# bharatlytics/faceRecognition_InfrenceEngine

Hardware: AMD Instinct MI355X
Metric: faces/sec end-to-end @1080p (higher is better)
Workload: dtype f16

## Files before the change

facerecognition_infrenceengine_amd/_lib.py:

```python
import ctypes as C
import struct
import os
import threading

_HERE = os.path.dirname(os.path.abspath(__file__))
LIB_PATH = os.path.join(_HERE, "csrc", "libfrhip.so")

_lock = threading.Lock()
_lib = None
ABI_VERSION = 106


class FrError(RuntimeError):
    pass


class ConvArgs(C.Structure):
    _fields_ = [("x", C.c_void_p), ("w", C.c_void_p), ("y", C.c_void_p),
                ("bias", C.c_void_p), ("slope", C.c_void_p), ("residual", C.c_void_p),
                ("out_f32_partial", C.c_void_p),
                ("B", C.c_int), ("H", C.c_int), ("W", C.c_int), ("Cin", C.c_int), ("Cout", C.c_int),
                ("KH", C.c_int), ("KW", C.c_int), ("stride", C.c_int), ("pad", C.c_int),
                ("Ho", C.c_int), ("Wo", C.c_int), ("bias_mode", C.c_int), ("splitk", C.c_int),
                ("x2", C.c_void_p), ("C2", C.c_int)]
# ... 63 lines not shown
    "fr_gallery_match_grouped_workspace": (_Z, [_I, _L]),
    "fr_gallery_match_grouped_f32": (_I, [_P, _P, _P, _P, _P, _I, _I, _L, _L, _I, _P, _P, _P, _Z, _P, _I, _P]),
    "fr_gallery_topk_grouped_workspace": (_Z, [_I, _L, _I]),
    "fr_gallery_topk_grouped_f32": (_I, [_P, _P, _P, _P, _P, _I, _I, _L, _L, _I, _I, _P, _P, _P, _Z, _P, _I, _P]),
    "fr_gallery_gmax_update": (_I, [_P, _P, _L, _I, _P, _P]),
    "fr_f32_to_f8": (_I, [_P, _P, _L, _P]),
    "fr_f32_to_f16": (_I, [_P, _P, _L, _P]),
    "fr_match_decide": (_I, [_P, _P, _I, _F, _F, _P, _P]),
    "fr_match_pack_candidates": (_I, [_P, _P, _I, _P, _P]),
    "fr_match_reduce_shards": (_I, [_P, _I, _I, _I, _I, _P, _P, _P]),
    "fr_match_reduce_shards_topk": (_I, [_P, _I, _I, _I, _I, _I, _P, _P, _P]),
    "fr_exchange_pack_queries": (_I, [_P, _I, _I, _I, _P, _P]),
    "fr_exchange_counts": (_I, [_P, _I, _I, _I, _P, _P]),
    "fr_gallery_first_above_f32": (_I, [_P, _P, _I, _L, _I, _F, _I, _L, _P, _P, _P, _Z, _P]),
    "fr_cosine_matrix_f32": (_I, [_P, _P, _I, _I, _I, _P, _P]),
    "fr_mean_rows_f32": (_I, [_P, _I, _I, _P, _P]),
    "fr_unknown_assign_batch_f32": (_I, [_P, _P, _I, _I, _F, _P, _P, _P, _I, _I, _P, _P, _P, _P]),
    "fr_gallery_first_above_blocked_f32": (_I, [_P, _P, _P, _P, _I, _L, _I, _F, _I, _L, _P, _P, _P, _Z, _P]),
    "fr_enrol_batch_workspace": (_Z, [_I, _L]),
    "fr_enrol_batch_f32": (_I, [_P, _P, _I, _P, _P, _I, _P, _I, _I, _I, _P, _P, _L, _F, _F, _P, _P, _P, _P, _P, _P, _P, _P,
                                _Z, _P]),
    "fr_gallery_pairs_workspace": (_Z, [_L, _L]),
    "fr_gallery_pairs_above_f16": (_I, [_P, _P, _L, _I, _F, _I, _L, _I, _P, _P, _P, _P, _Z, _P]),
    "fr_conv_nhwc_f16": (_I, [C.POINTER(ConvArgs), _P]),
    "fr_conv_sequence": (_I, [C.POINTER(ConvStep), _I, _P]),
    "fr_conv_inblock_f16": (_I, [C.POINTER(ConvArgs), _P]),
    "fr_conv_nhwc_f8": (_I, [C.POINTER(ConvF8Args), _P]),
    "fr_quantize_f16_f8": (_I, [_P, _P, _L, _F, _P]),
    "fr_quantize_f16_f8_centred": (_I, [_P, _P, _L, _I, _P, _F, _P]),
    "fr_gptq_round_e4m3": (_I, [_P, _P, _P, _P, _I, _I, _P]),
    "fr_conv_stage14_weight_bytes": (_Z, [_I]),
    "fr_conv_stage14_pack": (_I, [_P, _P, _P]),
    "fr_conv_stage14_f16": (_I, [_P, _P, _P, _P, _I, _I, _P]),
    "fr_conv_walk64_weight_bytes": (_Z, [_I]),
    "fr_conv_walk64_pack": (_I, [_P, _P, _I, _P]),
    "fr_conv_walk64_f16": (_I, [_P, _P, _P, _P, _I, _P, _P, _I, _I, _I, _P]),
    "fr_conv_stage28_weight_bytes": (_Z, [_I]),
    "fr_conv_stage28_pack": (_I, [_P, _P, _P]),
    "fr_conv_stage28_f16": (_I, [_P, _P, _P, _P, _I, _I, _P]),
    "fr_conv_stage14_f8_weight_bytes": (_Z, [_I]),
    "fr_conv_stage14_f8_param_floats": (_Z, []),
    "fr_conv_stage14_f8_pack": (_I, [_P, _P, _P]),
    "fr_conv_stage14_f8": (_I, [_P, _P, _P, _P, _P, _I, _I, _P]),
    "fr_conv_splitk_epilogue": (_I, [_P, _I, _I, _I, _I, _I, _P, _I, _P, _P, _P, _P]),
    "fr_fc_reduce_l2norm": (_I, [_P, _I, _I, _I, _P, _P, _P, _P]),
    "fr_warp_affine_5pt": (_I, [_P, _I, _I, _I, _P, _P, _P, _I, _I, _P, _P, _P, _P]),
    "fr_warp_affine_5pt_slots": (_I, [_P, _I, _I, _I, _P, _P, _I, _I, _P, _P]),
    "fr_warp_affine_5pt_refs": (_I, [_P, _I, _P, _P, _P, _I, _I, _P, _P, _P, _P]),
    "fr_warp_affine_5pt_slots_refs": (_I, [_P, _I, _P, _P, _I, _I, _P, _P]),
    "fr_letterbox_u8": (_I, [_P, _I, _P, _I, _I, _P]),
    "fr_detections_unscale": (_I, [_P, _P, _P, _P, _I, _I, _P]),
    "fr_yuv420_to_bgr_u8": (_I, [_P, _P, _I, _I, _I, _I, _I, _I, _I, _I, _I, _I, _P]),
    "fr_yuv420_to_bgr_refs_u8": (_I, [_P, _P, _I, _I, _I, _I, _I, _I, _I, _I, _P]),
    "fr_frame_activity_u8": (_I, [_P, _I, _I, _I, _P, _I, _P, _P, _P, _I, _P, _P, _P, _I, _I, _I, _P]),
    "fr_frame_activity_refs_u8": (_I, [_P, _I, _P, _I, _P, _P, _P, _I, _P, _P, _P, _I, _I, _I, _P]),
    "fr_track_associate_f32": (_I, [_P, _P, _P, _I, _I, _I, _I, _P, _P, _P, _F, _I, _I, _P, _P, _P, _P]),
    "fr_track_commit_f32": (_I, [_P, _P, _P, _P, _I, _I, _I, _I, _P, _P, _P, _P]),
    "fr_track_resolve_quality_i32": (_I, [_P, _P, _P, _P, _P, _P, _I, _I, _I, _I, _P, _P, _I, _P, _P, _P, _P]),
    "fr_track_fuse_f32": (_I, [_P, _P, _P, _P, _P, _P, _I, _I, _I, _I, _I, _F, _P, _P, _P, _P, _P, _P, _P]),
    "fr_face_quality_f16": (_I, [_P, _P, _P, _I, _I, _P, _P, _P, _F, _I, _I, _I, _I, _I, _F, _F, _F, _P]),
    "fr_pyramid_resize_norm":(_I, [_P, _I, _I, _I, _I, _I, _P, _P]),
    "fr_dconv_f32": (_I, [_P, _P, _P, _P, _P, _I, _I, _I, _I, _I, _I, _I, _I, _I, _P, _P, _I, _P]),
    "fr_dconv_mfma_f32": (_I, [_I, _P, _P, _P, _P, _P, _I, _I, _I, _P, _P, _P, _I, _I, _P, _I, _P, _P]),
    "fr_crop_conv1_f32": (_I, [_I, _P, _I, _I, _I, _P, _P, _I, _P, _P, _P, _P, _P]),
    "fr_crop_conv1_split": (_I, [_I, _P, _I, _I, _I, _P, _P, _I, _P, _P, _P, _P, _I, _P]),
    "fr_crop_conv1_list_f32": (_I, [_I, _P, _I, _I, _I, _P, _I, _P, _P, _I, _P, _P, _P, _P, _P]),
# ... 148 lines not shown
```

facerecognition_infrenceengine_amd/csrc/conv_stage14.hip:

```cpp
#include "common.h"
#include <type_traits>

namespace {

constexpr int S14_PX = 196, S14_C = 256, S14_ROWS = 200;
constexpr int S14_PLANE = S14_ROWS * 128;
constexpr int S14_IMG = 4 * S14_PLANE;
constexpr int S14_SLOT = 256 * 64;
constexpr int S14_PRM = 10 * 256 * 4;
constexpr int S14_LDS = S14_IMG + 3 * S14_SLOT + S14_PRM;
constexpr int S14_STEPS = 72;

struct StageP {
    const half_t* x;
    half_t* y;
    const half_t* w;
    const float* prm;
    int B, nconv;
    unsigned xbytes, wbytes;
};

}

__global__ __launch_bounds__(512, 2) void conv_stage14_kernel(StageP p) {
#if defined(__HIP_DEVICE_COMPILE__)
    extern __shared__ __attribute__((aligned(16))) char lds[];
    char* img = lds;
    char* ring = lds + S14_IMG;
    const float* lprm = reinterpret_cast<const float*>(lds + S14_IMG + 3 * S14_SLOT);
    const int tid = threadIdx.x, lane = tid & 63;
    const int wave = __builtin_amdgcn_readfirstlane(tid >> 6);
    const int wn = wave & 3, wp = wave >> 2;
    const int fr = lane & 15, fq = lane >> 4;
    const int n = blockIdx.x;
    const size_t img_elems = (size_t)S14_PX * S14_C;

    __amdgpu_buffer_rsrc_t wrs = buffer_rsrc(p.w, p.wbytes);
    __amdgpu_buffer_rsrc_t xrs = buffer_rsrc(p.x, p.xbytes);

    const unsigned wlane = (unsigned)(wave * 2048 + lane * 16);
    unsigned wsrc = 0;
    auto issue_w = [&](int slot) {
        char* dst = ring + slot * S14_SLOT + wave * 2048;
        __builtin_amdgcn_raw_ptr_buffer_load_lds(wrs, (lds_ptr_t)dst, 16, wlane, wsrc, 0, 0);
        __builtin_amdgcn_raw_ptr_buffer_load_lds(wrs, (lds_ptr_t)(dst + 1024), 16, wlane + 1024, wsrc, 0, 0);
        wsrc += S14_SLOT;
    };
    issue_w(0);
    issue_w(1);
    issue_w(2);
    __amdgpu_buffer_rsrc_t prs = buffer_rsrc(p.prm, (unsigned)p.nconv * S14_PRM);
    auto issue_prm = [&](int conv, int ln) {
        char* dst = lds + S14_IMG + 3 * S14_SLOT;
        __builtin_amdgcn_raw_ptr_buffer_load_lds(prs, (lds_ptr_t)(dst + wave * 1024), 16, (unsigned)(wave * 1024 + ln * 16), conv * S14_PRM, 0, 0);
        if (wave < 2)
            __builtin_amdgcn_raw_ptr_buffer_load_lds(prs, (lds_ptr_t)(dst + (8 + wave) * 1024), 16, (unsigned)((8 + wave) * 1024 + ln * 16), conv * S14_PRM, 0, 0);
    };

    {
        const int lrow = lane >> 3, ch = lane & 7;
        for (int pc = wave; pc < 100; pc += 8) {
            const int plane = pc / 25, row = (pc - plane * 25) * 8 + lrow;
            const unsigned off = row < S14_PX ? (unsigned)(((size_t)n * S14_PX + row) * 512 + plane * 128 + ((ch ^ (row & 7)) << 4))
                                              : 0x80000000u;
            __builtin_amdgcn_raw_ptr_buffer_load_lds(xrs, (lds_ptr_t)(img + plane * S14_PLANE + (pc - plane * 25) * 1024), 16, off, 0, 0, 0);
        }
    }

    auto run = [&](auto wp_tag) {
    constexpr int WP = decltype(wp_tag)::value;
    const int a_lane = fr * 64 + ((fq ^ (((fr >> 3) & 1) << 1)) << 4);
    const int a_own = wn * 4096 + a_lane;
    const int px0 = WP * 96 + fr;

    float4v acc[6][4], accx[2];
    int4v a0[4], a1[4], b[6], bx;
    int boff[7];

    int px0e = px0, fre = fr, fqe = fq;
    auto set_tap_one = [&](int j, int dy, int dx) {
        const int px = j < 6 ? px0e + 16 * j : 192 + fre;
        const int oy = px / 14, ox = px - oy * 14;
        const bool ok = px < S14_PX && (unsigned)(oy + dy) < 14u && (unsigned)(ox + dx) < 14u;
        const int pxn = ok ? px + dy * 14 + dx : S14_PX;
// ... 21 lines not shown
#pragma unroll
        for (int j = 0; j < 6; ++j) {
#pragma unroll
            for (int i = 0; i < 4; ++i) acc[j][i] = mfma16(ac[i], b[j], acc[j][i]);
            if (j == 0) { an[0] = rd_a(nslot, 0); an[1] = rd_a(nslot, 1); }
            if (j == 1) { an[2] = rd_a(nslot, 2); an[3] = rd_a(nslot, 3); }
            if (j == 2) {
                if (g == 7) { set_tap_one(6, dyn, dxn); set_tap_one(0, dyn, dxn); }
                bx = rd_b(ng, 6); b[0] = rd_b(ng, 0);
            }
            if (j == 3) {
                if (g == 7) { set_tap_one(1, dyn, dxn); set_tap_one(2, dyn, dxn); }
                b[1] = rd_b(ng, 1); b[2] = rd_b(ng, 2);
            }
            if (j == 4) {
                if (g == 7) { set_tap_one(3, dyn, dxn); set_tap_one(4, dyn, dxn); }
                b[3] = rd_b(ng, 3); b[4] = rd_b(ng, 4);
            }
            if (j == 5) {
                if (g == 7) set_tap_one(5, dyn, dxn);
                b[5] = rd_b(ng, 5);
            }
            FR_PIN();
            if constexpr (WP == 1) { if (j == 3) { issue_w(k % 3); FR_PIN(); } }
        }
    };

#pragma unroll
    for (int j = 0; j < 6; ++j)
#pragma unroll
        for (int i = 0; i < 4; ++i) acc[j][i] = float4v{0.f, 0.f, 0.f, 0.f};
    accx[0] = accx[1] = float4v{0.f, 0.f, 0.f, 0.f};
#pragma unroll 1
    for (int conv = 0; conv < p.nconv; ++conv) {
        int lane_e = lane;
        asm volatile("" : "+v"(lane_e));
        fre = lane_e & 15; fqe = lane_e >> 4; px0e = WP * 96 + fre;
        issue_prm(conv, lane_e);
        set_tap(-1, -1);
#pragma unroll
        for (int i = 0; i < 4; ++i) a0[i] = rd_a(0, i);
#pragma unroll
        for (int j = 0; j < 6; ++j) b[j] = rd_b(0, j);
        bx = rd_b(0, 6);
#pragma unroll 1
        for (int it = 0; it < 3; ++it) {
#pragma unroll
            for (int k = 0; k < 24; ++k) {
                asm volatile("s_waitcnt vmcnt(2) lgkmcnt(1)" ::: "memory");
                __builtin_amdgcn_s_barrier();
                FR_PIN();
                const int tt = k >> 3;
                const int dyn = tt < 2 ? it - 1 : it, dxn = tt < 2 ? tt : -1;
                if ((k & 1) == 0) step(a0, a1, k, dyn, dxn);
                else step(a1, a0, k, dyn, dxn);
            }
        }
        const bool second = conv & 1;
        half_t* ybase = p.y + (size_t)n * img_elems;
        asm volatile("" : "+v"(px0e), "+v"(fre), "+v"(fqe));
        asm volatile("s_waitcnt vmcnt(2)" ::: "memory");
        __builtin_amdgcn_s_barrier();
        int rowoff[7], key[7], clsoff[7];
#pragma unroll
        for (int j = 0; j < 7; ++j) {
            const int px = j < 6 ? px0e + 16 * j : 192 + fre;
            const int oy = (px * 4682) >> 16, ox = px - oy * 14;
            const int cls = (oy == 0 ? 0 : (oy >= 13 ? 2 : 1)) * 3 + (ox == 0 ? 0 : (ox == 13 ? 2 : 1));
            clsoff[j] = cls * S14_C;
            const int pxr = px < S14_PX ? px : S14_PX;
            rowoff[j] = wn * S14_PLANE + pxr * 128 + (fqe & 1) * 8;
            key[j] = pxr & 7;
        }
        const int co_own = wn * 64 + fqe * 4, co_sh = wn * 64 + WP * 32 + fqe * 4;
        const int ch_own = fqe >> 1, ch_sh = WP * 4 + (fqe >> 1);
        auto tiles = [&](auto prelu_tag) {
            constexpr bool FIRST = decltype(prelu_tag)::value;
            float4v sl[4], slx[2];
            if constexpr (FIRST) {
#pragma unroll
                for (int i = 0; i < 4; ++i) sl[i] = *reinterpret_cast<const float4v*>(lprm + 9 * S14_C + co_own + i * 16);
#pragma unroll
                for (int t = 0; t < 2; ++t) slx[t] = *reinterpret_cast<const float4v*>(lprm + 9 * S14_C + co_sh + t * 16);
            }
#pragma unroll
            for (int t = 0; t < 26; ++t) {
                float4v& a_ = t < 24 ? acc[t >> 2][t & 3] : accx[t - 24];
                const int j = t < 24 ? t >> 2 : 6, co = t < 24 ? co_own + (t & 3) * 16 : co_sh + (t - 24) * 16;
                const int ch = t < 24 ? ch_own + (t & 3) * 2 : ch_sh + (t - 24) * 2;
                half4* dst = reinterpret_cast<half4*>(img + rowoff[j] + ((ch ^ key[j]) << 4));
                float4v v = a_ + *reinterpret_cast<const float4v*>(lprm + clsoff[j] + co);
                if constexpr (FIRST) {
                    const half4 old = *dst;
                    const float4v s_ = t < 24 ? sl[t & 3] : slx[t - 24];
#pragma unroll
                    for (int e = 0; e < 4; ++e) v[e] = v[e] > 0.f ? v[e] : v[e] * s_[e];
                    a_ = float4v{(float)old[0], (float)old[1], (float)old[2], (float)old[3]};
                } else {
                    a_ = float4v{0.f, 0.f, 0.f, 0.f};
                }
                const half4 h = {(half_t)v[0], (half_t)v[1], (half_t)v[2], (half_t)v[3]};
                if (t < 24) *dst = h;
                else if (192 + fre < S14_PX) *dst = h;
                if ((t & 3) == 3) FR_PIN();
            }
        };
        if (second) tiles(std::false_type{}); else tiles(std::true_type{});
        asm volatile("s_waitcnt lgkmcnt(0)" ::: "memory");
        __builtin_amdgcn_s_barrier();
        if (conv == p.nconv - 1) {
            for (int e = tid; e < S14_PX * 32; e += 512) {
                const int px = e >> 5, c = e & 31;
                const int4v v = *reinterpret_cast<const int4v*>(img + (c >> 3) * S14_PLANE + px * 128 + (((c & 7) ^ (px & 7)) << 4));
                *reinterpret_cast<int4v*>(ybase + (size_t)px * S14_C + c * 8) = v;
            }
        }
    }
    };
    if (wp == 0) run(std::integral_constant<int, 0>{}); else run(std::integral_constant<int, 1>{});
    asm volatile("s_waitcnt vmcnt(0)" ::: "memory");
#endif
}

extern "C" size_t fr_conv_stage14_weight_bytes(int nconv) { return (size_t)(nconv > 0 ? nconv : 0) * S14_STEPS * S14_SLOT; }

__global__ void stage14_pack_weights(const half_t* __restrict__ w, half_t* __restrict__ out) {
    const int e = blockIdx.x * blockDim.x + threadIdx.x;
    if (e >= S14_STEPS * 256 * 4) return;
    const int q = e / 1024, r = e - q * 1024, row = r >> 2, cp = r & 3;
    const int chunk = cp ^ (((row >> 3) & 1) << 1);
    const int tap = q >> 3, g = q & 7;
    const int4v v = *reinterpret_cast<const int4v*>(w + (size_t)row * 2304 + tap * 256 + g * 32 + chunk * 8);
    *reinterpret_cast<int4v*>(out + (size_t)q * 8192 + row * 32 + cp * 8) = v;
}

extern "C" int fr_conv_stage14_pack(const void* w, void* out, fr_stream_t stream) {
    FR_REQUIRE(w && out, "fr_conv_stage14_pack: null pointer");
    stage14_pack_weights<<<fr_cdiv(S14_STEPS * 1024, 256), 256, 0, fr_stream(stream)>>>((const half_t*)w, (half_t*)out);
    FR_CHECK_LAUNCH("stage14_pack_weights");
    return FR_OK;
}

extern "C" int fr_conv_stage14_f16(const void* x, void* y, const void* wstream, const float* params, int B, int nblocks,
                                   fr_stream_t stream) {
    FR_REQUIRE(x && y && wstream && params && B > 0 && nblocks > 0, "fr_conv_stage14_f16: bad argument");
    FR_REQUIRE(x != y, "fr_conv_stage14_f16: x and y must be different buffers");
    FR_REQUIRE((int64_t)B * S14_PX * S14_C * 2 < (1ll << 31) && (int64_t)nblocks * 2 * S14_STEPS * S14_SLOT < (1ll << 32) - (1 << 20),
               "fr_conv_stage14_f16: tensor too large (B %d, blocks %d)", B, nblocks);
    StageP p;
    p.x = (const half_t*)x; p.y = (half_t*)y; p.w = (const half_t*)wstream; p.prm = params;
    p.B = B; p.nconv = 2 * nblocks;
    p.xbytes = (unsigned)((int64_t)B * S14_PX * S14_C * 2);
    p.wbytes = (unsigned)((int64_t)p.nconv * S14_STEPS * S14_SLOT);
    static FrDevLatch latch;
    if (!fr_raise_lds(reinterpret_cast<const void*>(conv_stage14_kernel), S14_LDS, latch)) {
        fr_set_error("fr_conv_stage14_f16: cannot raise dynamic LDS to %d bytes", S14_LDS);
        return FR_E_LAUNCH;
    }
    conv_stage14_kernel<<<B, 512, S14_LDS, fr_stream(stream)>>>(p);
    FR_CHECK_LAUNCH("conv_stage14_kernel");
    return FR_OK;
}
```

facerecognition_infrenceengine_amd/iresnet.py:

```python
import ctypes
import functools
import logging
import threading
import types
from collections import namedtuple

import torch

from . import _lib
from .weights import IRESNET_LAYERS, IRESNET_WIDTHS

BN_EPS = 1e-5
FC_SPLITK = 28
SMALL_BATCH = 48
INBLOCK_BATCH = 8
LOW_BATCH = 8
MAX_PLAN_STREAMS = 8
STAGE14_MIN_BATCH = 128
WALK64_SKIP = range(129, 160)
STAGE28_MIN_BATCH = 144


def _bn_fold(st, prefix, n, conv=None):
    if prefix + ".weight" in st:
        s = st[prefix + ".weight"].double() / torch.sqrt(st[prefix + ".running_var"].double() + BN_EPS)
        t = st[prefix + ".bias"].double() - st[prefix + ".running_mean"].double() * s
    else:
        s, t = torch.ones(n, dtype=torch.float64), torch.zeros(n, dtype=torch.float64)
    if conv is not None and conv + ".bias" in st:
        t = t + s * st[conv + ".bias"].double()
    return s, t


def _pack_w(w):
    return w.permute(0, 2, 3, 1).reshape(w.shape[0], -1).to(torch.float16).contiguous()


F8_MAX = 448.0
F8_MARGIN = 1.5


def f8_eligible(c, H):
    return c.k == 3 and c.stride == 1 and H in (14, 28) and c.cin % 128 == 0 and c.cout % 128 == 0


def round_e4m3(t):
    a = t.abs().clamp(max=F8_MAX)
    _, e = torch.frexp(a.clamp_min(2.0 ** -9))
    step = torch.ldexp(torch.ones_like(a), (e - 1).clamp_min(-6) - 3)
    return torch.copysign(torch.round(a / step) * step, t)

# ... 94 lines not shown
    run, best = [], []
    for i in range(nblocks):
        c1, c2 = convs[i, "c1"], convs[i, "c2"]
        ok = (i, "sc") not in convs and c1.cin == width and c1.cout == width and c2.stride == 1 and c2.cout == width
        run = run + [i] if ok else []
        if len(run) > len(best):
            best = run
    return (best[0], len(best)) if len(best) >= 2 else None


@functools.lru_cache(maxsize=None)
def conv_table(arch):
    R = ConvRec
    convs = {"stem": R("stem", 3, 1, 1, 8, 64, 0, 112, False, False, 0, 2 * 112 * 112 * 27 * 64)}
    cin, hw, bi = 64, 112, 0
    for n, cout in zip(IRESNET_LAYERS[arch], IRESNET_WIDTHS):
        for j in range(n):
            stride = 2 if j == 0 else 1
            ho = hw // stride
            fuses = j == 0 and cin % 64 == 0 and cout % 64 == 0
            convs[bi, "c1"] = R((bi, "c1"), 3, 1, 1, cin, cout, 1, hw, False, cin == 64 and cout % 64 == 0, 0, 2 * hw * hw * cin * cout * 9)
            convs[bi, "c2"] = R((bi, "c2"), 3, stride, 1, cout, cout, 0, hw, fuses, stride == 1 and cout == 64, 0, 2 * ho * ho * cout * cout * 9)
            if j == 0:
                convs[bi, "sc"] = R((bi, "sc"), 1, stride, 0, cin, cout, 0, hw, False, False, 0, 2 * ho * ho * cin * cout)
            if fuses:
                convs[bi, "fz"] = R((bi, "fz"), 3, stride, 1, cout, cout, 0, hw, False, False, cin, 2 * ho * ho * cout * (9 * cout + cin))
            cin, hw, bi = cout, ho, bi + 1
    convs["fc"] = R("fc", 1, 1, 0, 25088, 512, 0, 1, False, False, 0, 2 * 25088 * 512)
    flops = sum(c.flops for c in convs.values() if not c.c2)
    return ConvTable(arch, convs, bi, longest_run(convs, bi, 128), longest_run(convs, bi, 256), flops)


RouteMode = namedtuple("RouteMode", "small_batch low_batch inblock_batch use_stage14 use_stage28 use_walk64 fuse_shortcut fp8 "
                       "stage14_f8 profiled tapped calibrating",
                       defaults=(SMALL_BATCH, LOW_BATCH, INBLOCK_BATCH, True, True, True, True, frozenset(), False, False, False, False))
Step = namedtuple("Step", "route conv H W Ho Wo slices x2 src dst res want16 nxt tap variant flops")


def step_variant(route, c, H):
    if route in (STAGE28, STAGE14, STAGE14_F8):
        return {STAGE28: "conv_stage28_kernel", STAGE14: "conv_stage14_kernel<0, 0>", STAGE14_F8: "conv_stage14_f8_kernel<0>"}[route]
    if route == CONV_F8:
        return "conv_halo_kernel<2, 13, %d, 1, 4, false, true, 4, true, 8, 0>" % (256 if H == 14 else 320)
    if route == WALK64:
        return "conv_walk64_kernel %dx%d -> %d" % (H, H, c.cout)
    if route != PLAIN:
        return None
    if c.k == 3 and c.stride == 1 and c.cin % 64 == 0:
        if H in (7, 14, 28) and c.cout % 128 == 0:
            return "conv_halo_kernel<2, 13, %d, 1, 4, false, true, 4, false, 8, 0>" % {7: 384, 14: 256, 28: 320}[H]
        if H == 56 and c.cin == 64:
            return "conv_halo_kernel<1, 14, 384, 1, 4, false, false, 4, false, 8, 0>"
        if H == 112 and c.cin == 64 and c.cout == 64:
            return "conv_halo_kernel<1, 14, 512, 1, 4, false, false, 4, false, 8, 0>"
    return "conv_stem_kernel<112>" if c.cin == 8 else "conv_mfma_kernel<%d, false, true>" % (2 if c.cout % 128 == 0 else 1)


def step_cost(table, route, conv, B):
    run = route in (STAGE28, STAGE14, STAGE14_F8)
    c = table.convs[(conv[0], "c1") if run else conv]
    return step_variant(route, c, c.H), float(B * c.flops * (2 * conv[1] if run else 1))


def conv_step(table, B, mode, rules, key, src, dst, res=None, x2=False, tap=None):
    c = table.convs[key]
    Ho = (c.H + 2 * c.pad - c.k) // c.stride + 1
    route, slices = PLAIN, 1
    if key == "fc":
# ... 37 lines not shown
            if run is run14 and fp8:
                if not h8:
                    steps.append(special(QUANTISE, k1, H, "h", "h"))
                h8 = False
            steps.append(special(STAGE28 if run is run28 else STAGE14_F8 if fp8 else STAGE14, run, H, "h", "h"))
            bi += run[1]
            continue
        li += 1 if entry else 0
        tap = "layer%d.0.mid" % li if entry else None
        if f1:
            if not h8:
                steps.append(special(QUANTISE, k1, H, "h", "h"))
            steps.append(special(CONV_F8, k1, H, "h", "mid", want16=not f2 or mode.tapped, nxt=k2 if f2 else None, tap=tap))
        else:
            steps.append(conv(k1, "h", "mid", tap=tap))
        fz = mode.fuse_shortcut and not f2 and cv[k2].fuses
        if entry and not fz:
            steps.append(conv(ksc, "h", "short"))
        res = "short" if entry else "h"
        if fz:
            steps.append(conv((bi, "fz"), "mid", "h", x2=True))
        elif f2:
            if not f1:
                steps.append(special(QUANTISE, k2, H, "mid", "mid"))
            steps.append(special(CONV_F8, k2, H, "mid", "h", res, nxt=n1 if n1 in fp8 else None))
        else:
            steps.append(conv(k2, "mid", "h", res))
        h8 = f2 and not fz and n1 in fp8
        bi += 1
    steps.append(conv("fc", "h", "emb"))
    return tuple(steps)


class _Conv:
    __slots__ = ("key", "w", "bias", "slope", "cin", "cout", "k", "stride", "pad", "bias_mode", "w32", "w8", "sw", "sx",
                 "oscale", "mu", "bias8", "c2", "w64")

    def __init__(self, rec, w, bias, slope, device):
        self.key, self.k, self.stride, self.pad, self.cin, self.cout, self.bias_mode = rec[:7]
        self.c2 = rec.c2
        self.w = w.to(device)
        self.w32 = self.w8 = self.sw = self.sx = self.oscale = self.mu = self.bias8 = None
        self.bias = None if bias is None else bias.to(torch.float32).contiguous().to(device)
        self.slope = None if slope is None else slope.to(torch.float32).contiguous().to(device)
        self.w64 = None


class IResNetHIP:

    def __init__(self, state, arch="r100", device="cuda:0", max_chunk=256, small_batch=SMALL_BATCH, low_batch=LOW_BATCH,
                 inblock_batch=INBLOCK_BATCH):
        _lib.require_gpu()
        self.small_batch, self.low_batch, self.inblock_batch = int(small_batch), int(low_batch), int(inblock_batch)
        self.lib = _lib.load()
        self.device = torch.device(device)
        self.arch = arch
        self.max_chunk = max_chunk
        dev = self.device
        f = fold_iresnet(state, arch)
        self.table = conv_table(arch)
        rec, cv = self.table.convs, {}
        self._convs = cv
        self.stem = cv["stem"] = _Conv(rec["stem"], f["stem"]["w"].to(torch.float16).contiguous(), f["stem"]["bias"], f["stem"]["slope"], dev)
        self.blocks = []
        self.fused_sc = {}
        self.fuse_shortcut = True
        for i, b in enumerate(f["blocks"]):
            d1, d2, ds = b["c1"], b["c2"], b["sc"]
            c1 = cv[i, "c1"] = _Conv(rec[i, "c1"], _pack_w(d1["w"]), d1["bias"], d1["slope"], dev)
            c2 = cv[i, "c2"] = _Conv(rec[i, "c2"], _pack_w(d2["w"]), d2["bias"], None, dev)
            if d1["cin"] % 128 == 0 and d1["cout"] % 128 == 0:
                c1.w32 = d1["w"].permute(0, 2, 3, 1).reshape(d1["cout"], -1).to(torch.float32)
            if d2["stride"] == 1 and d2["cout"] % 128 == 0:
                c2.w32 = d2["w"].permute(0, 2, 3, 1).reshape(d2["cout"], -1).to(torch.float32)
            sc = None
            if ds is not None:
                sc = cv[i, "sc"] = _Conv(rec[i, "sc"], _pack_w(ds["w"]), ds["bias"], None, dev)
            if (i, "fz") in rec:
                w = torch.cat([c2.w.reshape(c2.cout, -1), sc.w.reshape(sc.cout, -1)], 1).contiguous()
                self.fused_sc[i] = cv[i, "fz"] = _Conv(rec[i, "fz"], w, c2.bias + sc.bias, None, dev)
            self.blocks.append((c1, c2, sc))
        self.fc = cv["fc"] = _Conv(rec["fc"], f["fc_w"].to(torch.float16).contiguous(), None, None, dev)
        self.fc_bias = f["fc_bias"].to(torch.float32).contiguous().to(dev)
        self.stage14 = self._pack_stage(self.table.run14, 14)
        self.stage28 = self._pack_stage(self.table.run28, 28)
        self._pack_walk64()
        self.flops_per_face = self.table.flops_per_face
        self._routes = {}
        self._plans = {}
        self._plan_bufs = {}
        self._plan_lock = threading.Lock()
        self._plan_limit_logged = False
        self.profile = None
        self.fp8, self._fp8_keys = False, frozenset()
        self.use_stage28 = self.use_stage14 = True
        self.stage14_f8 = None
        self._calib = None

    def _pack_stage(self, run, hw):
        if run is None:
            return None
        first, n = run
        width = self.blocks[first][0].cin
        pack = getattr(self.lib, "fr_conv_stage%d_pack" % hw)
        per = getattr(self.lib, "fr_conv_stage%d_weight_bytes" % hw)(1) // 2
        stream = torch.empty(2 * n * per, dtype=torch.float16, device=self.device)
        prm = torch.empty((2 * n, 10, width), dtype=torch.float32, device=self.device)
        with torch.cuda.device(self.device):
            for k, c in enumerate(c for b in self.blocks[first:first + n] for c in b[:2]):
                pack(_lib.ptr(c.w), _lib.ptr(stream[k * per:]), _lib.stream_ptr())
                prm[k, :9] = c.bias.reshape(9, width) if c.bias_mode == 1 else c.bias[None, :]
                prm[k, 9] = c.slope if c.slope is not None else 1.0
            torch.cuda.synchronize(self.device)
        return {"first": first, "n": n, "w": stream, "prm": prm.contiguous()}

    def _pack_walk64(self):
        self.use_walk64 = True
        with torch.cuda.device(self.device):
            for key, c in self._convs.items():
                if self.table.convs[key].walk64:
                    c.w64 = torch.empty(self.lib.fr_conv_walk64_weight_bytes(c.cout) // 2, dtype=torch.float16, device=self.device)
                    self.lib.fr_conv_walk64_pack(_lib.ptr(c.w), _lib.ptr(c.w64), c.cout, _lib.stream_ptr())
            torch.cuda.synchronize(self.device)

    def _run_stage(self, s, h):
        st, fn = (self.stage28, self.lib.fr_conv_stage28_f16) if s.route == STAGE28 else (self.stage14, self.lib.fr_conv_stage14_f16)
        y = torch.empty_like(h)
        self._launch(fn, (_lib.ptr(h), _lib.ptr(y), _lib.ptr(st["w"]), _lib.ptr(st["prm"]), h.shape[0], s.conv[1], _lib.stream_ptr()),
                     s.variant, s.flops)
        return h if s.route == STAGE28 else y

    def fp8_candidates(self):
        sized = [(c, self.table.convs[c.key].H) for b in self.blocks for c in b[:2]]
        return [(c, hw) for c, hw in sized if c.w32 is not None and f8_eligible(c, hw)]

    def enable_fp8(self, calib_crops, select="accurate", centre=True, gptq=True):
        assert calib_crops.dtype == torch.float16 and calib_crops.shape[1:] == (112, 112, 8)
        cands = self.fp8_candidates()
        if select == "all":
            chosen = [c for c, _ in cands]
        elif select == "accurate":
            chosen = [c for c, hw in cands if hw == 14] + [c for c, hw in cands if hw == 28][-4:]
        else:
            chosen = [c for i, (c, _) in enumerate(cands) if select(i, len(cands))]
        self.fp8 = False
        for c, _ in cands:
            c.oscale = None
        self._calib = {"want": {id(c) for c in chosen}, "centre": centre, "gptq": gptq, "stats": {}}
        self.forward(calib_crops.contiguous())
        stats, self._calib = self._calib["stats"], None
        n = 0
        for c in chosen:
            st = stats.get(id(c))
            if st is None:
                continue
            c.sx = max(st["absmax"] * F8_MARGIN / F8_MAX, 1e-12)
            c.mu = st["mu"]
            w8, sw = quantise_weights_f8(c.w32)
            if st.get("wq") is not None:
                w8 = st["wq"].cpu().to(torch.float8_e4m3fn).view(torch.uint8).contiguous()
            c.w8, c.sw = w8.to(self.device), sw.to(self.device)
            c.oscale = (c.sw * c.sx).contiguous()
            base = c.bias.double().cpu()
# ... 113 lines not shown
        fn(*args)
        e1.record()
        self.profile.append((variant, flops, e0, e1))

    @staticmethod
    def _conv_args(s, c, B, x, y, residual, partial, x2):
        return _lib.ConvArgs(_lib.ptr(x), _lib.ptr(c.w), _lib.ptr(y), _lib.ptr(c.bias), _lib.ptr(c.slope), _lib.ptr(residual),
                             _lib.ptr(partial), B, s.H, s.W, c.cin, c.cout, c.k, c.k, c.stride, c.pad, s.Ho, s.Wo, c.bias_mode,
                             s.slices, _lib.ptr(x2), c.c2 if x2 is not None else 0)

    def _issue(self, s, c, x, residual=None, x2=None, partial=None):
        B, stream = x.shape[0], _lib.stream_ptr()
        y = None if partial is not None else torch.empty((B, s.Ho, s.Wo, c.cout), dtype=torch.float16, device=self.device)
        if s.route == WALK64:
            self._launch(self.lib.fr_conv_walk64_f16, (_lib.ptr(x), _lib.ptr(c.w64), _lib.ptr(y), _lib.ptr(c.bias), c.bias_mode,
                                                       _lib.ptr(c.slope), _lib.ptr(residual), B, s.H, c.cout, stream), s.variant, s.flops)
        elif s.route == SPLITK:
            M = B * s.Ho * s.Wo
            part = torch.empty((s.slices, M, c.cout), dtype=torch.float32, device=self.device)
            a = _lib.ConvArgs(_lib.ptr(x), _lib.ptr(c.w), None, None, None, None, _lib.ptr(part), B, s.H, s.W, c.cin, c.cout,
                              c.k, c.k, c.stride, c.pad, s.Ho, s.Wo, 0, s.slices, _lib.ptr(x2), c.c2)
            self.lib.fr_conv_nhwc_f16(ctypes.byref(a), stream)
            self.lib.fr_conv_splitk_epilogue(_lib.ptr(part), s.slices, M, c.cout, s.Ho, s.Wo, _lib.ptr(c.bias), c.bias_mode,
                                             _lib.ptr(c.slope), _lib.ptr(residual), _lib.ptr(y), stream)
        else:
            a = self._conv_args(s, c, B, x, y, residual, partial, x2)
            self._launch(self.lib.fr_conv_inblock_f16 if s.route == INBLOCK else self.lib.fr_conv_nhwc_f16,
                         (ctypes.byref(a), stream), s.variant, s.flops)
        return y

    def _mode(self, taps=None):
        return RouteMode(self.small_batch, self.low_batch, self.inblock_batch, self.use_stage14, self.use_stage28,
                         self.use_walk64, self.fuse_shortcut, self._fp8_keys if self.fp8 else frozenset(),
                         self.stage14_f8 is not None, self.profile is not None, taps is not None, self._calib is not None)

    def _conv(self, x, c, B, H, W, residual=None, x2=None):
        s = conv_step(self.table, B, self._mode(), self, c.key, "x", "h", x2=x2 is not None)
        assert (H, W) == (s.H, s.W)
        return self._issue(s, c, x, residual, x2), s.Ho, s.Wo

    def forward(self, x, taps=None):
        assert x.dtype == torch.float16 and x.shape[1:] == (112, 112, 8) and x.is_contiguous()
        B = x.shape[0]
        emb = torch.empty((B, 512), dtype=torch.float32, device=self.device)
        normed = torch.empty_like(emb)
        with torch.cuda.device(self.device):
            for b0 in range(0, B, self.max_chunk):
                b1 = min(B, b0 + self.max_chunk)
                self._forward_chunk(x[b0:b1], emb[b0:b1], normed[b0:b1], taps)
        return emb, normed

    def _splitk_floats(self, route, B):
        return max([s.slices * B * s.Ho * s.Wo * self.table.convs[s.conv].cout for s in route if s.route == SPLITK] + [1])

    def release_plans(self):
        with self._plan_lock:
            self._plans.clear()
            self._plan_bufs.clear()
            self._plan_limit_logged = False

    def _plan(self, B, mode, route):
        sid = torch.cuda.current_stream(self.device).cuda_stream
        key = (B, sid)
        plan = self._plans.get(key)
        if plan is not None:
            return plan
        if any(s.route not in _SEQ_KIND for s in route[:-1]):
# ... 20 lines not shown
            buf = free.pop()
            if s.dst == "h":
                free += [own.pop(name) for name in ("h", "mid", "short") if name in own]
            own[s.dst] = buf
            x, residual, x2 = t[s.src], t.get(s.res), t["h"] if s.x2 else None
            t[s.dst] = y = buf[:B * s.Ho * s.Wo * c.cout].view(B, s.Ho, s.Wo, c.cout)
            st.kind = _SEQ_KIND[s.route]
            st.args = self._conv_args(s, c, B, x, y, residual, partial if s.route == SPLITK else None, x2)
        plan = self._plans[key] = (arr, len(arr), t["h"], bufs, partial)
        return plan

    def _route(self, B, mode):
        route = self._routes.get((B, mode))
        if route is None:
            route = self._routes[B, mode] = embed_route(self.table, B, mode, self)
        return route

    def _forward_chunk(self, x, emb, normed, taps):
        B = x.shape[0]
        mode = self._mode(taps)
        route = self._route(B, mode)
        plan = None
        if B <= self.low_batch and not (mode.profiled or mode.tapped or mode.calibrating or mode.fp8):
            with self._plan_lock:
                plan = self._plan(B, mode, route)
        if plan is not None:
            arr, n, h, _, _ = plan
            with self._plan_lock:
                arr[0].args.x = x.data_ptr()
                self.lib.fr_conv_sequence(arr, n, _lib.stream_ptr())
                self._fc(route[-1], h, emb, normed)
            return
        t, t8 = {"x": x}, {}
        for s in route[:-1]:
            if s.route == QUANTISE:
                t8[s.src] = self._quantise(t[s.src], self._convs[s.conv])
            elif s.route == STAGE14_F8:
                t["h"] = self._run_stage14_f8(t["h"], t8["h"], B)
            elif s.route == STAGE28 or s.route == STAGE14:
                t["h"] = self._run_stage(s, t["h"])
            elif s.route == CONV_F8:
                y, y8 = self._conv_f8(t8[s.src], self._convs[s.conv], B, s.H, s.W, residual=t.get(s.res), want16=s.want16,
                                      nxt=self._convs.get(s.nxt))
                t[s.dst], t8[s.dst] = y, y8
            else:
                c, xs = self._convs[s.conv], t[s.src]
                if mode.calibrating:
                    self._calib_observe(c, xs, s.H)
                t[s.dst] = self._issue(s, c, xs, t.get(s.res), t["h"] if s.x2 else None)
            if taps is not None and s.tap is not None:
                taps[s.tap] = t[s.dst]
        if taps is not None:
            taps["final"] = t["h"]
        self._fc(route[-1], t["h"], emb, normed)

    def _fc(self, s, h, emb, normed):
        B = h.shape[0]
        partial = torch.empty((FC_SPLITK, B, 512), dtype=torch.float32, device=self.device)
        self._issue(s, self.fc, h, partial=partial)
        self.lib.fr_fc_reduce_l2norm(_lib.ptr(partial), FC_SPLITK, B, 512, _lib.ptr(self.fc_bias),
                                     _lib.ptr(emb), _lib.ptr(normed), _lib.stream_ptr())
```

include/frhip.h:

```cpp
#ifndef FRHIP_H
#define FRHIP_H
#include <stddef.h>
#include <stdint.h>
#ifdef __cplusplus
extern "C" {
#endif

#define FR_OK 0
#define FR_E_INVALID (-1)
#define FR_E_LAUNCH (-2)
#define FR_E_NODEVICE (-3)

typedef void* fr_stream_t;

#define FR_ABI_VERSION 106
int fr_version(void);
const char* fr_last_error_string(void);
int fr_device_count(void);

int fr_l2norm_rows_f32(const float* x, float* out, int rows, int dim, fr_stream_t stream);

size_t fr_gallery_match_workspace(int F, int64_t N);
int fr_gallery_match_f32(const float* Q, const float* G, int F, int64_t N, int D,
                         int64_t row_offset, int64_t* out_idx, float* out_score,
// ... 105 lines not shown
                       float sim_thr, float dup_thr, int32_t* status, int32_t* pair, int32_t* face, float* avg, float* row,
                       int64_t* dup_pos, float* dup_score, void* workspace, size_t workspace_bytes, fr_stream_t stream);
#define FR_PAIRS_OVERFLOW 1
#define FR_PAIRS_NONFINITE 2
size_t fr_gallery_pairs_workspace(int64_t N, int64_t capacity);
int fr_gallery_pairs_above_f16(const float* G32, const int64_t* view, int64_t N, int D, float thr, int inclusive,
                               int64_t capacity, int max_ranges, int64_t* out_key, float* out_score, int32_t* out_counts,
                               void* workspace, size_t workspace_bytes, fr_stream_t stream);

typedef struct {
    const void* x; const void* w; void* y;
    const float* bias; const float* slope; const void* residual;
    float* out_f32_partial;
    int B, H, W, Cin, Cout, KH, KW, stride, pad, Ho, Wo;
    int bias_mode; int splitk;
    const void* x2; int C2;
} fr_conv_args;
int fr_conv_nhwc_f16(const fr_conv_args* args, fr_stream_t stream);
typedef struct {
    const void* x8; const void* w8; void* y16; void* y8;
    const float* oscale; const float* bias; const float* slope; const void* residual;
    int B, H, W, Cin, Cout, bias_mode;
    float y8_mul;
    const float* y8_sub;
} fr_conv_f8_args;
int fr_conv_nhwc_f8(const fr_conv_f8_args* args, fr_stream_t stream);
int fr_quantize_f16_f8(const void* x16, void* out8, int64_t n, float mul, fr_stream_t stream);
int fr_quantize_f16_f8_centred(const void* x16, void* out8, int64_t n, int C, const float* sub, float mul,
                               fr_stream_t stream);
size_t fr_conv_stage14_weight_bytes(int nconv);
int fr_conv_stage14_pack(const void* w, void* out, fr_stream_t stream);
int fr_conv_stage14_f16(const void* x, void* y, const void* wstream, const float* params, int B, int nblocks,
                        fr_stream_t stream);
size_t fr_conv_stage28_weight_bytes(int nconv);
int fr_conv_stage28_pack(const void* w, void* out, fr_stream_t stream);
int fr_conv_stage28_f16(void* x, void* mid, const void* wstream, const float* params, int B, int nblocks, fr_stream_t stream);
size_t fr_conv_walk64_weight_bytes(int Cout);
int fr_conv_walk64_pack(const void* w, void* out, int Cout, fr_stream_t stream);
int fr_conv_walk64_f16(const void* x, const void* wstream, void* y, const float* bias, int bias_mode, const float* slope,
                       const void* residual, int B, int HW, int Cout, fr_stream_t stream);
size_t fr_conv_stage14_f8_weight_bytes(int nconv);
size_t fr_conv_stage14_f8_param_floats(void);
int fr_conv_stage14_f8_pack(const void* w8, void* out, fr_stream_t stream);
int fr_conv_stage14_f8(const void* x8, const void* x16, void* y16, const void* wstream, const float* params, int B,
                       int nblocks, fr_stream_t stream);
int fr_gptq_round_e4m3(const double* W, const double* U, const float* sw, float* Q, int rows, int K, fr_stream_t stream);
int fr_conv_splitk_epilogue(const float* partial, int splitk, int M, int Cout, int Ho, int Wo,
                            const float* bias, int bias_mode, const float* slope, const void* residual,
                            void* y, fr_stream_t stream);
int fr_conv_inblock_f16(const fr_conv_args* args, fr_stream_t stream);
typedef struct {
    int kind;
    fr_conv_args args;
} fr_conv_step;
int fr_conv_sequence(const fr_conv_step* steps, int nsteps, fr_stream_t stream);
int fr_fc_reduce_l2norm(const float* partial, int splitk, int B, int dim, const float* bias,
                        float* embedding, float* normed, fr_stream_t stream);


int fr_warp_affine_5pt(const uint8_t* frames, int nframes, int H, int W, const float* kps,
                       const int32_t* frame_idx, const int32_t* count, int F, int size,
                       void* out_f16_nhwc8, uint8_t* out_u8_bgr, float* M_out, fr_stream_t stream);

int fr_warp_affine_5pt_slots(const uint8_t* frames, int nframes, int H, int W, const float* kps,
                             const int32_t* counts, int cap, int size, void* out_f16_nhwc8,
                             fr_stream_t stream);
// ... 167 lines not shown
```

Baseline: 27030.

## Fuse next-stage 3x3 conv into persistent stage14 kernel as tail convs

Result: slower. 26740 (-1.1%).

```diff
diff --git a/facerecognition_infrenceengine_amd/_lib.py b/facerecognition_infrenceengine_amd/_lib.py
--- a/facerecognition_infrenceengine_amd/_lib.py
+++ b/facerecognition_infrenceengine_amd/_lib.py
@@ -119,6 +119,8 @@
     "fr_conv_stage14_weight_bytes": (_Z, [_I]),
     "fr_conv_stage14_pack": (_I, [_P, _P, _P]),
     "fr_conv_stage14_f16": (_I, [_P, _P, _P, _P, _I, _I, _P]),
+    "fr_conv_stage14_pack_tail": (_I, [_P, _P, _P]),
+    "fr_conv_stage14_ext_f16": (_I, [_P, _P, _P, _P, _P, _I, _I, _P]),
     "fr_conv_walk64_weight_bytes": (_Z, [_I]),
     "fr_conv_walk64_pack": (_I, [_P, _P, _I, _P]),
     "fr_conv_walk64_f16": (_I, [_P, _P, _P, _P, _I, _P, _P, _I, _I, _I, _P]),
diff --git a/facerecognition_infrenceengine_amd/csrc/conv_stage14.hip b/facerecognition_infrenceengine_amd/csrc/conv_stage14.hip
--- a/facerecognition_infrenceengine_amd/csrc/conv_stage14.hip
+++ b/facerecognition_infrenceengine_amd/csrc/conv_stage14.hip
@@ -11,6 +11,8 @@
 constexpr int S14_LDS = S14_IMG + 3 * S14_SLOT + S14_PRM;
 constexpr int S14_STEPS = 72;
 
+typedef unsigned uint4v __attribute__((ext_vector_type(4)));
+
 struct StageP {
     const half_t* x;
     half_t* y;
@@ -18,10 +20,12 @@
     const float* prm;
     int B, nconv;
     unsigned xbytes, wbytes;
+    half_t* ytail;
 };
 
 }
 
+template <bool TAIL>
 __global__ __launch_bounds__(512, 2) void conv_stage14_kernel(StageP p) {
 #if defined(__HIP_DEVICE_COMPILE__)
     extern __shared__ __attribute__((aligned(16))) char lds[];
@@ -49,7 +53,9 @@
     issue_w(0);
     issue_w(1);
     issue_w(2);
-    __amdgpu_buffer_rsrc_t prs = buffer_rsrc(p.prm, (unsigned)p.nconv * S14_PRM);
+    constexpr int NTAIL = TAIL ? 2 : 0;
+    __amdgpu_buffer_rsrc_t prs = buffer_rsrc(p.prm, (unsigned)(p.nconv + NTAIL) * S14_PRM);
+    half_t* tbase = TAIL ? p.ytail + (size_t)n * (S14_PX * 512) : nullptr;
     auto issue_prm = [&](int conv, int ln) {
         char* dst = lds + S14_IMG + 3 * S14_SLOT;
         __builtin_amdgcn_raw_ptr_buffer_load_lds(prs, (lds_ptr_t)(dst + wave * 1024), 16, (unsigned)(wave * 1024 + ln * 16), conv * S14_PRM, 0, 0);
@@ -137,7 +143,7 @@
         for (int i = 0; i < 4; ++i) acc[j][i] = float4v{0.f, 0.f, 0.f, 0.f};
     accx[0] = accx[1] = float4v{0.f, 0.f, 0.f, 0.f};
 #pragma unroll 1
-    for (int conv = 0; conv < p.nconv; ++conv) {
+    for (int conv = 0; conv < p.nconv + NTAIL; ++conv) {
         int lane_e = lane;
         asm volatile("" : "+v"(lane_e));
         fre = lane_e & 15; fqe = lane_e >> 4; px0e = WP * 96 + fre;
@@ -178,6 +184,46 @@
             key[j] = pxr & 7;
         }
         const int co_own = wn * 64 + fqe * 4, co_sh = wn * 64 + WP * 32 + fqe * 4;
+        if constexpr (TAIL) {
+            if (conv >= p.nconv) {
+                asm volatile("" : "+s"(tbase));
+                __amdgpu_buffer_rsrc_t trs = buffer_rsrc(tbase, S14_PX * 1024u);
+                const unsigned tface = (unsigned)(conv - p.nconv) * 512u;
+                const unsigned co8 = (unsigned)(wn * 64 + (fqe & 1) * 16 + (fqe >> 1) * 8) * 2u;
+                float4v sl[4];
+#pragma unroll
+                for (int i = 0; i < 4; ++i) sl[i] = *reinterpret_cast<const float4v*>(lprm + 9 * S14_C + co_own + i * 16);
+                auto act = [&](float4v& a_, int j, int co, const float4v& s_) {
+                    float4v v = a_ + *reinterpret_cast<const float4v*>(lprm + clsoff[j] + co);
+#pragma unroll
+                    for (int e = 0; e < 4; ++e) v[e] = v[e] > 0.f ? v[e] : v[e] * s_[e];
+                    a_ = float4v{0.f, 0.f, 0.f, 0.f};
+                    return __builtin_bit_cast(int2v, half4{(half_t)v[0], (half_t)v[1], (half_t)v[2], (half_t)v[3]});
+                };
+                auto put = [&](int2v pa, int2v pb, unsigned off) {
+                    const auto s0 = __builtin_amdgcn_permlane16_swap((unsigned)pa[0], (unsigned)pb[0], false, false);
+                    const auto s1 = __builtin_amdgcn_permlane16_swap((unsigned)pa[1], (unsigned)pb[1], false, false);
+                    __builtin_amdgcn_raw_buffer_store_b128(uint4v{s0[0], s1[0], s0[1], s1[1]}, trs, off, 0, 0);
+                };
+#pragma unroll
+                for (int j = 0; j < 6; ++j) {
+#pragma unroll
+                    for (int ip = 0; ip < 2; ++ip) {
+                        const int2v pa = act(acc[j][2 * ip], j, co_own + ip * 32, sl[2 * ip]);
+                        const int2v pb = act(acc[j][2 * ip + 1], j, co_own + ip * 32 + 16, sl[2 * ip + 1]);
+                        put(pa, pb, tface + (unsigned)(px0e + 16 * j) * 1024u + co8 + ip * 64u);
+                    }
+                    FR_PIN();
+                }
+                {
+                    const int2v pa = act(accx[0], 6, co_sh, sl[2 * WP]), pb = act(accx[1], 6, co_sh + 16, sl[2 * WP + 1]);
+                    put(pa, pb, 192 + fre < S14_PX ? tface + (unsigned)(192 + fre) * 1024u + co8 + WP * 64u : 0x80000000u);
+                }
+                asm volatile("s_waitcnt vmcnt(0) lgkmcnt(0)" ::: "memory");
+                __builtin_amdgcn_s_barrier();
+                continue;
+            }
+        }
         const int ch_own = fqe >> 1, ch_sh = WP * 4 + (fqe >> 1);
         auto tiles = [&](auto prelu_tag) {
             constexpr bool FIRST = decltype(prelu_tag)::value;
@@ -219,10 +265,18 @@
                 const int4v v = *reinterpret_cast<const int4v*>(img + (c >> 3) * S14_PLANE + px * 128 + (((c & 7) ^ (px & 7)) << 4));
                 *reinterpret_cast<int4v*>(ybase + (size_t)px * S14_C + c * 8) = v;
             }
-        }
-    }
-    };
-    if (wp == 0) run(std::integral_constant<int, 0>{}); else run(std::integral_constant<int, 1>{});
+            if constexpr (TAIL) asm volatile("s_waitcnt vmcnt(0)" ::: "memory");
+        }
+    }
+    };
+    if constexpr (TAIL) {
+        int wps = wp;
+        if (wps != 0) run(std::integral_constant<int, 1>{});
+        asm volatile("" : "+s"(wps));
+        if (wps == 0) run(std::integral_constant<int, 0>{});
+    } else {
+        if (wp == 0) run(std::integral_constant<int, 0>{}); else run(std::integral_constant<int, 1>{});
+    }
     asm volatile("s_waitcnt vmcnt(0)" ::: "memory");
 #endif
 }
@@ -246,23 +300,49 @@
     return FR_OK;
 }
 
+extern "C" int fr_conv_stage14_pack_tail(const void* w, void* out, fr_stream_t stream) {
+    FR_REQUIRE(w && out, "fr_conv_stage14_pack_tail: null pointer");
+    for (int hf = 0; hf < 2; ++hf) {
+        stage14_pack_weights<<<fr_cdiv(S14_STEPS * 1024, 256), 256, 0, fr_stream(stream)>>>(
+            (const half_t*)w + (size_t)hf * 256 * 2304, (half_t*)out + (size_t)hf * S14_STEPS * 8192);
+        FR_CHECK_LAUNCH("stage14_pack_weights");
+    }
+    return FR_OK;
+}
+
+static int stage14_launch(const char* who, const void* x, void* y, void* ytail, const void* wstream, const float* params, int B,
+                          int nblocks, fr_stream_t stream) {
+    const int nall = 2 * nblocks + (ytail ? 2 : 0);
+    FR_REQUIRE((int64_t)B * S14_PX * (ytail ? 512 : S14_C) * 2 < (1ll << 31) && (int64_t)nall * S14_STEPS * S14_SLOT < (1ll << 32) - (1 << 20),
+               "%s: tensor too large (B %d, blocks %d)", who, B, nblocks);
+    StageP p;
+    p.x = (const half_t*)x; p.y = (half_t*)y; p.w = (const half_t*)wstream; p.prm = params;
+    p.B = B; p.nconv = 2 * nblocks;
+    p.xbytes = (unsigned)((int64_t)B * S14_PX * S14_C * 2);
+    p.wbytes = (unsigned)((int64_t)nall * S14_STEPS * S14_SLOT);
+    p.ytail = (half_t*)ytail;
+    static FrDevLatch latch[2];
+    const void* fn = ytail ? reinterpret_cast<const void*>(conv_stage14_kernel<true>) : reinterpret_cast<const void*>(conv_stage14_kernel<false>);
+    if (!fr_raise_lds(fn, S14_LDS, latch[ytail != nullptr])) {
+        fr_set_error("%s: cannot raise dynamic LDS to %d bytes", who, S14_LDS);
+        return FR_E_LAUNCH;
+    }
+    if (ytail) conv_stage14_kernel<true><<<B, 512, S14_LDS, fr_stream(stream)>>>(p);
+    else conv_stage14_kernel<false><<<B, 512, S14_LDS, fr_stream(stream)>>>(p);
+    FR_CHECK_LAUNCH("conv_stage14_kernel");
+    return FR_OK;
+}
+
 extern "C" int fr_conv_stage14_f16(const void* x, void* y, const void* wstream, const float* params, int B, int nblocks,
                                    fr_stream_t stream) {
     FR_REQUIRE(x && y && wstream && params && B > 0 && nblocks > 0, "fr_conv_stage14_f16: bad argument");
     FR_REQUIRE(x != y, "fr_conv_stage14_f16: x and y must be different buffers");
-    FR_REQUIRE((int64_t)B * S14_PX * S14_C * 2 < (1ll << 31) && (int64_t)nblocks * 2 * S14_STEPS * S14_SLOT < (1ll << 32) - (1 << 20),
-               "fr_conv_stage14_f16: tensor too large (B %d, blocks %d)", B, nblocks);
-    StageP p;
-    p.x = (const half_t*)x; p.y = (half_t*)y; p.w = (const half_t*)wstream; p.prm = params;
-    p.B = B; p.nconv = 2 * nblocks;
-    p.xbytes = (unsigned)((int64_t)B * S14_PX * S14_C * 2);
-    p.wbytes = (unsigned)((int64_t)p.nconv * S14_STEPS * S14_SLOT);
-    static FrDevLatch latch;
-    if (!fr_raise_lds(reinterpret_cast<const void*>(conv_stage14_kernel), S14_LDS, latch)) {
-        fr_set_error("fr_conv_stage14_f16: cannot raise dynamic LDS to %d bytes", S14_LDS);
-        return FR_E_LAUNCH;
-    }
-    conv_stage14_kernel<<<B, 512, S14_LDS, fr_stream(stream)>>>(p);
-    FR_CHECK_LAUNCH("conv_stage14_kernel");
-    return FR_OK;
-}
+    return stage14_launch("fr_conv_stage14_f16", x, y, nullptr, wstream, params, B, nblocks, stream);
+}
+
+extern "C" int fr_conv_stage14_ext_f16(const void* x, void* y, void* ytail, const void* wstream, const float* params, int B,
+                                       int nblocks, fr_stream_t stream) {
+    FR_REQUIRE(x && y && ytail && wstream && params && B > 0 && nblocks > 0, "fr_conv_stage14_ext_f16: bad argument");
+    FR_REQUIRE(x != y && ytail != x && ytail != y, "fr_conv_stage14_ext_f16: x, y and ytail must be different buffers");
+    return stage14_launch("fr_conv_stage14_ext_f16", x, y, ytail, wstream, params, B, nblocks, stream);
+}
diff --git a/facerecognition_infrenceengine_amd/iresnet.py b/facerecognition_infrenceengine_amd/iresnet.py
--- a/facerecognition_infrenceengine_amd/iresnet.py
+++ b/facerecognition_infrenceengine_amd/iresnet.py
@@ -17,6 +17,7 @@
 LOW_BATCH = 8
 MAX_PLAN_STREAMS = 8
 STAGE14_MIN_BATCH = 128
+STAGE14_TAIL_MIN_BATCH = 224
 WALK64_SKIP = range(129, 160)
 STAGE28_MIN_BATCH = 144
 
@@ -177,8 +178,8 @@
 
 
 RouteMode = namedtuple("RouteMode", "small_batch low_batch inblock_batch use_stage14 use_stage28 use_walk64 fuse_shortcut fp8 "
-                       "stage14_f8 profiled tapped calibrating",
-                       defaults=(SMALL_BATCH, LOW_BATCH, INBLOCK_BATCH, True, True, True, True, frozenset(), False, False, False, False))
+                       "stage14_f8 profiled tapped calibrating use_stage14_tail",
+                       defaults=(SMALL_BATCH, LOW_BATCH, INBLOCK_BATCH, True, True, True, True, frozenset(), False, False, False, False, True))
 Step = namedtuple("Step", "route conv H W Ho Wo slices x2 src dst res want16 nxt tap variant flops")
 
 
@@ -282,6 +283,16 @@
     return tuple(steps)
 
 
+def stage14_tail(table, route, i, B, mode):
+    if STAGE14_TAIL_MIN_BATCH is None or B < STAGE14_TAIL_MIN_BATCH or not mode.use_stage14_tail or mode.profiled:
+        return False
+    s, t = route[i], route[i + 1]
+    if s.route != STAGE14 or t.route != PLAIN or t.conv != (s.conv[0] + s.conv[1], "c1") or t.src != "h" or t.x2:
+        return False
+    c = table.convs[t.conv]
+    return (c.k, c.stride, c.pad, c.cin, c.cout, c.bias_mode, c.H) == (3, 1, 1, 256, 512, 1, 14)
+
+
 class _Conv:
     __slots__ = ("key", "w", "bias", "slope", "cin", "cout", "k", "stride", "pad", "bias_mode", "w32", "w8", "sw", "sx",
                  "oscale", "mu", "bias8", "c2", "w64")
@@ -344,6 +355,7 @@
         self.profile = None
         self.fp8, self._fp8_keys = False, frozenset()
         self.use_stage28 = self.use_stage14 = True
+        self.use_stage14_tail = True
         self.stage14_f8 = None
         self._calib = None
 
@@ -354,15 +366,26 @@
         width = self.blocks[first][0].cin
         pack = getattr(self.lib, "fr_conv_stage%d_pack" % hw)
         per = getattr(self.lib, "fr_conv_stage%d_weight_bytes" % hw)(1) // 2
-        stream = torch.empty(2 * n * per, dtype=torch.float16, device=self.device)
-        prm = torch.empty((2 * n, 10, width), dtype=torch.float32, device=self.device)
+        tail = self._convs.get((first + n, "c1")) if hw == 14 else None
+        if tail is not None and (tail.k, tail.stride, tail.cin, tail.cout, tail.bias_mode) != (3, 1, 256, 512, 1):
+            tail = None
+        nall = 2 * n + (2 if tail is not None else 0)
+        stream = torch.empty(nall * per, dtype=torch.float16, device=self.device)
+        prm = torch.empty((nall, 10, width), dtype=torch.float32, device=self.device)
         with torch.cuda.device(self.device):
             for k, c in enumerate(c for b in self.blocks[first:first + n] for c in b[:2]):
                 pack(_lib.ptr(c.w), _lib.ptr(stream[k * per:]), _lib.stream_ptr())
                 prm[k, :9] = c.bias.reshape(9, width) if c.bias_mode == 1 else c.bias[None, :]
                 prm[k, 9] = c.slope if c.slope is not None else 1.0
+            if tail is not None:
+                self.lib.fr_conv_stage14_pack_tail(_lib.ptr(tail.w), _lib.ptr(stream[2 * n * per:]), _lib.stream_ptr())
+                prm[2 * n:, :9] = tail.bias.reshape(9, 2, width).permute(1, 0, 2)
+                prm[2 * n:, 9] = tail.slope.reshape(2, width)
             torch.cuda.synchronize(self.device)
-        return {"first": first, "n": n, "w": stream, "prm": prm.contiguous()}
+        st = {"first": first, "n": n, "w": stream[:2 * n * per], "prm": prm[:2 * n]}
+        if tail is not None:
+            st.update(w_ext=stream, prm_ext=prm)
+        return st
 
     def _pack_walk64(self):
         self.use_walk64 = True
@@ -379,6 +402,15 @@
         self._launch(fn, (_lib.ptr(h), _lib.ptr(y), _lib.ptr(st["w"]), _lib.ptr(st["prm"]), h.shape[0], s.conv[1], _lib.stream_ptr()),
                      s.variant, s.flops)
         return h if s.route == STAGE28 else y
+
+    def _run_stage14_tail(self, s, t, h):
+        st, B = self.stage14, h.shape[0]
+        y = torch.empty_like(h)
+        ytail = torch.empty((B, t.Ho, t.Wo, 512), dtype=torch.float16, device=self.device)
+        self._launch(self.lib.fr_conv_stage14_ext_f16, (_lib.ptr(h), _lib.ptr(y), _lib.ptr(ytail), _lib.ptr(st["w_ext"]),
+                                                        _lib.ptr(st["prm_ext"]), B, s.conv[1], _lib.stream_ptr()),
+                     s.variant, s.flops + t.flops)
+        return y, ytail
 
     def fp8_candidates(self):
         sized = [(c, self.table.convs[c.key].H) for b in self.blocks for c in b[:2]]
@@ -558,7 +590,8 @@
     def _mode(self, taps=None):
         return RouteMode(self.small_batch, self.low_batch, self.inblock_batch, self.use_stage14, self.use_stage28,
                          self.use_walk64, self.fuse_shortcut, self._fp8_keys if self.fp8 else frozenset(),
-                         self.stage14_f8 is not None, self.profile is not None, taps is not None, self._calib is not None)
+                         self.stage14_f8 is not None, self.profile is not None, taps is not None, self._calib is not None,
+                         self.use_stage14_tail)
 
     def _conv(self, x, c, B, H, W, residual=None, x2=None):
         s = conv_step(self.table, B, self._mode(), self, c.key, "x", "h", x2=x2 is not None)
@@ -645,8 +678,14 @@
                 self._fc(route[-1], h, emb, normed)
             return
         t, t8 = {"x": x}, {}
-        for s in route[:-1]:
-            if s.route == QUANTISE:
+        fused = None
+        for i, s in enumerate(route[:-1]):
+            if s is fused:
+                continue
+            if s.route == STAGE14 and "w_ext" in self.stage14 and stage14_tail(self.table, route, i, B, mode):
+                fused = route[i + 1]
+                t["h"], t[fused.dst] = self._run_stage14_tail(s, fused, t["h"])
+            elif s.route == QUANTISE:
                 t8[s.src] = self._quantise(t[s.src], self._convs[s.conv])
             elif s.route == STAGE14_F8:
                 t["h"] = self._run_stage14_f8(t["h"], t8["h"], B)
diff --git a/include/frhip.h b/include/frhip.h
--- a/include/frhip.h
+++ b/include/frhip.h
@@ -161,6 +161,9 @@
 int fr_conv_stage14_pack(const void* w, void* out, fr_stream_t stream);
 int fr_conv_stage14_f16(const void* x, void* y, const void* wstream, const float* params, int B, int nblocks,
                         fr_stream_t stream);
+int fr_conv_stage14_pack_tail(const void* w, void* out, fr_stream_t stream);
+int fr_conv_stage14_ext_f16(const void* x, void* y, void* ytail, const void* wstream, const float* params, int B,
+                            int nblocks, fr_stream_t stream);
 size_t fr_conv_stage28_weight_bytes(int nconv);
 int fr_conv_stage28_pack(const void* w, void* out, fr_stream_t stream);
 int fr_conv_stage28_f16(void* x, void* mid, const void* wstream, const float* params, int B, int nblocks, fr_stream_t stream);
```
